# sovrasov/3d-object-detection.pytorch

Measured on AMD Instinct MI355X. Metric: regression train crops/sec @224^2 bs256 MobileNetV2, higher is better.
Workload: dtype bf16; 1 GPU; mobilenetv2 9-class Objectron keypoint regression, train step (fwd + l1/add/CE losses + bwd + AdamW), 224x224 crops, per-GPU batch 256; global_batch=256, parallelism=dp1, roofline_sampled_steps=0, rccl_ranks=0

## Files before the change

3d-object-detection.pytorch_amd/csrc/elementwise.hip:

```cpp
#include "common.h"

namespace {

template <typename T, bool U8>
__global__ __launch_bounds__(256) void im2col_kernel(const void* __restrict__ xin, const float* __restrict__ mean,
                                                     const float* __restrict__ istd, T* __restrict__ col, int B,
                                                     int H, int W, int Ho, int Wo) {
  extern __shared__ float tile[];
  const int WP = W + 2;
  const int hp = (Ho + 1) / 2;
  const int b = blockIdx.x / hp, oy0 = (blockIdx.x % hp) * 2;
  const int iy0 = oy0 * 2 - 1;
  const int tid = threadIdx.x;
  for (int i = tid; i < 15 * 2; i += 256) {
    const int rr = i >> 1;
    tile[rr * WP + ((i & 1) ? W + 1 : 0)] = 0.f;
  }
  if constexpr (U8) {
    const unsigned char* xu = reinterpret_cast<const unsigned char*>(xin);
    const float mu[3] = {mean[0], mean[1], mean[2]}, is[3] = {istd[0], istd[1], istd[2]};
    const int RB = W * 3;
    if ((RB & 3) == 0) {
      const int R4 = RB >> 2;
      for (int i = tid; i < 5 * R4; i += 256) {
// ... 245 lines not shown
template <typename T>
__global__ __launch_bounds__(256) void gap_fwd_kernel(const EwArgs a) {
  __shared__ float red[8 * 32 * 8];
  __shared__ float redm[8 * 32 * 8];
  __shared__ int redi[8 * 32 * 8];
  const int CG = a.C / 8, b = blockIdx.x;
  const int cgs = pool_cgs(CG), nslots = 256 / cgs, rowl = cgs * 8;
  const int cgl = threadIdx.x & (cgs - 1), slot = threadIdx.x / cgs;
  const int cg = blockIdx.y * cgs + cgl;
  const bool on = cg < CG;
  const int c0 = on ? cg * 8 : 0;
  const bool want_max = a.mode != T3D_POOL_AVG;
  const T* __restrict__ y = reinterpret_cast<const T*>(a.a);
  float sc[8], sh[8], acc[8], mx[8];
  int mi[8];
  load_affine(a, c0, sc, sh);
#pragma unroll
  for (int j = 0; j < 8; ++j) { acc[j] = 0.f; mx[j] = -INFINITY; mi[j] = 0; }
  if (on) {
    for (int hw = slot; hw < a.HW; hw += nslots) {
      float v[8];
      Vec8<T>::load(y + ((size_t)b * a.HW + hw) * a.C + c0, v);
      act_affine_vec<8>(v, sc, sh, a.act);
#pragma unroll
      for (int j = 0; j < 8; ++j) {
        acc[j] += v[j];
        if (v[j] > mx[j]) { mx[j] = v[j]; mi[j] = hw; }
      }
    }
  }
#pragma unroll
// ... 203 lines not shown
  else return T3D_ERR_ARG;
  T3D_CHECK_LAUNCH();
  return T3D_OK;
}

extern "C" int t3d_pool_fwd(int dtype, const void* y, const t3d_prologue* pro, int mode, float* pooled, int* argmax,
                            int B, int HW, int C, void* stream) {
  if (!y || !pooled || B <= 0 || HW <= 0 || C <= 0 || (C % 8)) return T3D_ERR_ARG;
  if (mode != T3D_POOL_AVG && mode != T3D_POOL_MAX && mode != T3D_POOL_AVGMAX) return T3D_ERR_ARG;
  if (pro && pro->se) return T3D_ERR_UNSUPPORTED;
  EwArgs a{};
  a.a = y; a.pooled = pooled; a.C = C; a.HW = HW; a.inv_hw = 1.f / (float)HW; a.mode = mode; a.argmax = argmax;
  fill_pro(a, pro);
  dim3 grid(B, cdiv(C / 8, 32));
  hipStream_t st = reinterpret_cast<hipStream_t>(stream);
  if (const int rc = t3d_fold_fallback(a.scale, st)) return rc;
  if (dtype == T3D_F32) T3D_LAUNCH(gap_fwd_kernel<float>, grid, dim3(256), 0, st, a);
  else if (dtype == T3D_BF16) T3D_LAUNCH(gap_fwd_kernel<bf16_t>, grid, dim3(256), 0, st, a);
  else if (dtype == T3D_F16) T3D_LAUNCH(gap_fwd_kernel<f16_t>, grid, dim3(256), 0, st, a);
  else return T3D_ERR_ARG;
  T3D_CHECK_LAUNCH();
  return T3D_OK;
}

extern "C" int t3d_gap_fwd(int dtype, const void* y, const t3d_prologue* pro, float* pooled, int B, int HW, int C,
                           void* stream) {
  return t3d_pool_fwd(dtype, y, pro, T3D_POOL_AVG, pooled, nullptr, B, HW, C, stream);
}

extern "C" int t3d_pool_bwd(int dtype, const float* dpooled, const void* y, const t3d_prologue* pro, int mode,
                            const int* argmax, void* dz, double* stats, int B, int HW, int C, void* stream) {
// ... 22 lines not shown
```

3d-object-detection.pytorch_amd/csrc/plan.hip:

```cpp
#include <chrono>
#include <cstdio>
#include <cstdlib>
#include <cstring>
#include <string>
#include <utility>
#include <vector>

#include "common.h"

namespace {

template <class T>
inline T word_to(uint64_t v) {
  if constexpr (std::is_pointer<T>::value) {
    return reinterpret_cast<T>(static_cast<uintptr_t>(v));
  } else if constexpr (std::is_same<T, float>::value) {
    const uint32_t b = static_cast<uint32_t>(v);
    float f;
    std::memcpy(&f, &b, 4);
    return f;
  } else if constexpr (std::is_same<T, double>::value) {
    double d;
    std::memcpy(&d, &v, 8);
    return d;
// ... 12 lines not shown

template <auto Fn>
struct Thunk;
template <class... A, int (*Fn)(A...)>
struct Thunk<Fn> {
  static int run(const uint64_t* w) { return call_words(Fn, w, std::index_sequence_for<A...>{}); }
};

struct Entry { const char* name; int (*run)(const uint64_t*); int nargs; };
#define T3D_E(fn) {#fn, &Thunk<&fn>::run, arity(&fn)}
const Entry kEntries[] = {
    T3D_E(t3d_dwconv_fwd), T3D_E(t3d_bn_finalize), T3D_E(t3d_bn_eval_affine), T3D_E(t3d_bn_eval_affine_batched),
    T3D_E(t3d_pwconv_fwd), T3D_E(t3d_pwconv_dgrad), T3D_E(t3d_pack_weight), T3D_E(t3d_sum_replicas_batched),
    T3D_E(t3d_set_dw_slots), T3D_E(t3d_set_exact_pool), T3D_E(t3d_sum_slots_batched), T3D_E(t3d_dwconv_bwd),
    T3D_E(t3d_pwconv_wgrad), T3D_E(t3d_pwconv_yfree_prep), T3D_E(t3d_pwconv_dgrad_yfree), T3D_E(t3d_pwconv_wgrad_yfree),
    T3D_E(t3d_pwconv_yfree_prep2), T3D_E(t3d_pwconv_bwd_yfree), T3D_E(t3d_pwconv_bwd_yfree_w), T3D_E(t3d_pwconv_wgrad_yfree_finish),
    T3D_E(t3d_bn_bwd_finalize), T3D_E(t3d_stem_im2col), T3D_E(t3d_stem_im2col_u8), T3D_E(t3d_crop_resize_u8),
    T3D_E(t3d_pwconv_fwd_mat), T3D_E(t3d_im2col), T3D_E(t3d_im2col_nchw), T3D_E(t3d_col2im_bwd), T3D_E(t3d_pack_conv_weight),
    T3D_E(t3d_unpack_conv_grad), T3D_E(t3d_maxpool_fwd), T3D_E(t3d_maxpool_bwd), T3D_E(t3d_res_relu_fwd),
    T3D_E(t3d_res_relu_bwd), T3D_E(t3d_subsample), T3D_E(t3d_ir_block_eval), T3D_E(t3d_bn_apply), T3D_E(t3d_bn_act_bwd),
    T3D_E(t3d_gap_fwd), T3D_E(t3d_gap_bwd), T3D_E(t3d_pool_fwd), T3D_E(t3d_pool_bwd), T3D_E(t3d_head_fwd),
    T3D_E(t3d_linear_fwd), T3D_E(t3d_head_fwd_all), T3D_E(t3d_head_bwd), T3D_E(t3d_head_bwd_weights), T3D_E(t3d_se_fwd),
    T3D_E(t3d_se_bwd), T3D_E(t3d_se_fwd_fused), T3D_E(t3d_se_bwd_data), T3D_E(t3d_se_bwd_weights), T3D_E(t3d_se_after_sums),
    T3D_E(t3d_se_after_apply), T3D_E(t3d_se_after_bwd), T3D_E(t3d_set_reduction_replicas), T3D_E(t3d_set_workspace), T3D_E(t3d_set_main_workspace),
    T3D_E(t3d_fold_request), T3D_E(t3d_pack_weights_batched), T3D_E(t3d_pwconv_pack_frag), T3D_E(t3d_adamw_step), T3D_E(t3d_set_grad_watch),
    T3D_E(t3d_sgd_step), T3D_E(t3d_rmsprop_step), T3D_E(t3d_adadelta_step),
    T3D_E(t3d_zero_batched), T3D_E(t3d_copy_cols), T3D_E(t3d_bn_bias_grad), T3D_E(t3d_se_bwd_affine), T3D_E(t3d_dropout_mask),
    T3D_E(t3d_loss_fwd_bwd), T3D_E(t3d_metrics_per_sample), T3D_E(t3d_iou3d), T3D_E(t3d_box_iou3d), T3D_E(t3d_ssd_decode_nms),
    T3D_E(t3d_expdw_fwd), T3D_E(t3d_track_step), T3D_E(t3d_ssd_select_rects), T3D_E(t3d_head_select), T3D_E(t3d_track_kp_to_frame),
};
// ... 247 lines not shown
```

3d-object-detection.pytorch_amd/csrc/pwconv_common.h:

```cpp
#pragma once
#include "common.h"

namespace t3d_pw {

struct GemmArgs {
  const void* a0;
  const void* a1;
  const float *p0, *p1, *p2;
  int act, se_after, per_sample, dgrad;
  const void* w;
  const float* bias;
  const void* e_y;
  const float *e_scale, *e_shift, *e_se;
  int e_act, e_se_after;
  const void* e_res;
  void* out;
  double* stats;
  float* ps_stats;
  int ps_wave;
  int M, HW, Kin, Nout, mtiles;
  int kz;
  float* part;
  const void* a2;
  int Kin2, ks1;
  int row0;
  const T3dFold* fold;
  const void* z_res;
  void* z_out;
  int unused_[8];
  int wfrag;
  T3dQuant quant;
};

template <typename T> __device__ __forceinline__ void ldvec(const T* p, float* v);
template <> __device__ __forceinline__ void ldvec<float>(const float* p, float* v) {
  const float4 a = *reinterpret_cast<const float4*>(p);
  v[0] = a.x; v[1] = a.y; v[2] = a.z; v[3] = a.w;
}
template <> __device__ __forceinline__ void ldvec<bf16_t>(const bf16_t* p, float* v) { Vec8<bf16_t>::load(p, v); }
template <typename T> __device__ __forceinline__ void stvec(T* p, const float* v);
template <> __device__ __forceinline__ void stvec<float>(float* p, const float* v) {
  *reinterpret_cast<float4*>(p) = make_float4(v[0], v[1], v[2], v[3]);
}
template <> __device__ __forceinline__ void stvec<bf16_t>(bf16_t* p, const float* v) { Vec8<bf16_t>::store(p, v); }
// ... 10 lines not shown
```

3d-object-detection.pytorch_amd/csrc/pwconv_stream.hip:

```cpp
#include <cstdlib>
#include <type_traits>
#include "pwconv_common.h"

#ifndef T3D_PW_F16
typedef bf16_t ST;
typedef bf16x8 ST8;
#define T3D_PW_MFMA __builtin_amdgcn_mfma_f32_16x16x32_bf16
#define T3D_PW_LAUNCH stream_launch
#else
typedef f16_t ST;
typedef f16x8 ST8;
#define T3D_PW_MFMA __builtin_amdgcn_mfma_f32_16x16x32_f16
#define T3D_PW_LAUNCH stream_launch_f16
#endif

namespace t3d_pw {
__device__ __forceinline__ f32x2 pk_fma_clamp01(f32x2 a, f32x2 b, f32x2 c) {
  f32x2 d;
  asm("v_pk_fma_f32 %0, %1, %2, %3 clamp" : "=v"(d) : "v"(a), "v"(b), "v"(c));
  return d;
}

namespace {


#ifdef T3D_PW_TRACE
__device__ unsigned long long g_pw_trace[16];
#define PW_STAMP(i)                                                                                       \
  do {                                                                                                    \
    if (threadIdx.x == 0 && (blockIdx.x == 0 || blockIdx.x == gridDim.x - 1))                            \
      g_pw_trace[(blockIdx.x == 0 ? 0 : 8) + (i)] = wall_clock64();                                       \
  } while (0)
#else
#define PW_STAMP(i)
#endif

template <int NT, int R, bool DG, bool GEN, bool YF = false, int KU = 2, bool ZM = false>
__global__ __launch_bounds__(512, KU > 2 ? 1 : 2) void pw_stream_kernel(const GemmArgs a, const int nchunks, const int KS, const int nrep, const long long rstride) {
  constexpr int BN = NT * 16;
  extern __shared__ __attribute__((aligned(16))) unsigned char smem[];
  ST8* Wf = reinterpret_cast<ST8*>(smem);
  const int kpad = KS * 32;
  float* coef = reinterpret_cast<float*>(smem + (size_t)NT * KS * 1024);
  float* lstat = coef + 3 * kpad;
  float* ecoef = lstat + BN * 2;
  double* dstat = reinterpret_cast<double*>(ecoef + 2 * BN);

  const int tid = threadIdx.x, lane = tid & 63, wave = tid >> 6;
  const int lg = lane >> 4, lc = lane & 15;
  const int nxb = gridDim.x / nchunks;
  int chunk, xb;
  if (nchunks > 1 && (nxb & 7) == 0) {
    const int xcd = blockIdx.x & 7, j = blockIdx.x >> 3;
    chunk = j % nchunks;
    xb = (j / nchunks) * 8 + xcd;
  } else {
    chunk = blockIdx.x % nchunks;
    xb = blockIdx.x / nchunks;
  }
  const int n0 = chunk * BN;
  const ST* __restrict__ A0 = reinterpret_cast<const ST*>(a.a0);
  const ST* __restrict__ A1 = reinterpret_cast<const ST*>(a.a1);
  const ST* __restrict__ A2 = reinterpret_cast<const ST*>(a.a2);
  const int ks1 = A2 ? a.ks1 : (1 << 30);
  const ST* __restrict__ Wg = reinterpret_cast<const ST*>(a.w);
  ST* __restrict__ out = reinterpret_cast<ST*>(a.out);
  PW_STAMP(0);

  const int nthr = blockDim.x, WAVES = nthr >> 6;
  auto stage_weights = [&]() {
  if (a.wfrag) {
    constexpr int SU = 8;
    const int total = NT * KS * 64, tiles = (a.Nout + 31) / 32 * 2, t0 = n0 / 16;
    const ST8* __restrict__ P = reinterpret_cast<const ST8*>(a.w) + (size_t)t0 * KS * 64;
    const int valid = max(0, min(NT, tiles - t0)) * KS * 64;
    for (int i0 = tid; i0 < total; i0 += nthr * SU) {
      ST8 v[SU];
#pragma unroll
      for (int u = 0; u < SU; ++u) v[u] = P[min(i0 + u * nthr, valid - 1)];
#pragma unroll
      for (int u = 0; u < SU; ++u) {
        const int i = i0 + u * nthr;
        if (i >= valid) {
#pragma unroll
// ... 14 lines not shown
        const int l = i & 63, ks = (i >> 6) % KS, t = (i >> 6) / KS;
        const int n = n0 + (t >> 1) * 32 + ((l & 15) >> 2) * 8 + (t & 1) * 4 + (l & 3), k = ks * 32 + (l >> 4) * 8;
        ok[u] = n < a.Nout && k < a.Kin;
        v[u] = *reinterpret_cast<const ST8*>(Wg + (size_t)min(n, a.Nout - 1) * a.Kin + min(k, a.Kin - 8));
      }
#pragma unroll
      for (int u = 0; u < SU; ++u) {
        if (!ok[u]) {
#pragma unroll
          for (int j = 0; j < 8; ++j) v[u][j] = (ST)0.f;
        }
        if (i0 + u * nthr < total) Wf[i0 + u * nthr] = v[u];
      }
    }
  }
  for (int i = tid; i < BN * 2; i += nthr) { lstat[i] = 0.f; dstat[i] = 0.0; }
  for (int i = tid; i < BN; i += nthr) {
    const int n = n0 + i;
    const bool v = DG && a.e_scale && n < a.Nout;
    ecoef[i] = v ? a.e_scale[n] : 1.f;
    ecoef[BN + i] = v ? a.e_shift[n] : 0.f;
  }
  };
  constexpr bool DGL = DG && !YF;
  if (!YF && a.fold) {
    for (int i = a.Kin + tid; i < kpad; i += nthr) {
      coef[i] = DG ? 0.f : 1.f; coef[kpad + i] = 0.f; coef[2 * kpad + i] = 0.f;
    }
    t3d_fold_block(a.fold, 0, a.Kin, coef, kpad, blockIdx.x == 0, stage_weights);
  } else {
  stage_weights();
  for (int i = tid; i < kpad; i += nthr) {
    const bool v = i < a.Kin;
    if (YF) {
      coef[i] = 1.f; coef[kpad + i] = 0.f; coef[2 * kpad + i] = 0.f;
    } else if (!DG) {
      coef[i] = (v && a.p0) ? a.p0[i] : 1.f;
      coef[kpad + i] = (v && a.p0) ? a.p1[i] : 0.f;
    } else {
      coef[i] = (v && !a.per_sample) ? a.p0[i] : 0.f;
// ... 220 lines not shown
            err[q] = *reinterpret_cast<const ST8*>(reinterpret_cast<const ST*>(a.e_res) + (size_t)mld[r] * a.Nout +
                                                      min(nb + 32 * q, a.Nout - 8));
        }
      }
#pragma unroll
      for (int q = 0; q < NT / 2; ++q) {
        const int n = nb + 32 * q;
        if (n >= a.Nout) continue;
        float v[8], yv[8];
#pragma unroll
        for (int j = 0; j < 8; ++j) v[j] = acc[r][2 * q + (j >> 2)][j & 3];
        if (c6f) {
#pragma unroll
          for (int j = 0; j < 8; ++j) v[j] *= 6.f;
        }
        if ((!DG || YF) && a.bias) {
#pragma unroll
          for (int j = 0; j < 8; ++j) v[j] += a.bias[n + j];
        }
        if (DG && a.e_y) {
#pragma unroll
          for (int j = 0; j < 8; ++j) yv[j] = (float)eyr[q][j];
          if (GEN && a.e_se) {
            const float4 s0 = *reinterpret_cast<const float4*>(ecoef + (n - n0)), s1 = *reinterpret_cast<const float4*>(ecoef + (n - n0) + 4);
            const float4 h0 = *reinterpret_cast<const float4*>(ecoef + BN + (n - n0)),
                         h1 = *reinterpret_cast<const float4*>(ecoef + BN + (n - n0) + 4);
            float es[8] = {s0.x, s0.y, s0.z, s0.w, s1.x, s1.y, s1.z, s1.w};
            float eh[8] = {h0.x, h0.y, h0.z, h0.w, h1.x, h1.y, h1.z, h1.w};
            const float4 g0 = esg[GEN ? q : 0][0], g1 = esg[GEN ? q : 0][1];
            const float sv[8] = {g0.x, g0.y, g0.z, g0.w, g1.x, g1.y, g1.z, g1.w};
            if (!a.e_se_after) {
// ... 93 lines not shown
        if (lc == 0 && n < a.Nout) {
          atomicAdd(dstat + (n - n0 + j) * 2, t3d_snap(s1, a.quant, false));
          atomicAdd(dstat + (n - n0 + j) * 2 + 1, t3d_snap(s2, a.quant, !DG));
        }
      }
    }
    __syncthreads();
    for (int i = tid; i < BN * 2; i += nthr) {
      const int n = n0 + (i >> 1);
      if (n < a.Nout) atomicAdd(a.stats + (size_t)(xb % nrep) * rstride + (size_t)(i & 1) * a.Nout + n, dstat[i]);
    }
  }
  PW_STAMP(4);
}

template <int NT, int R, bool DG, bool GEN, bool YF = false, int KU = 2, bool ZM = false>
int launch_v(GemmArgs& a, int KS, hipStream_t st) {
  constexpr int BN = NT * 16;
  const int kpad = KS * 32;
  const size_t lds = (size_t)NT * KS * 1024 + (size_t)3 * kpad * 4 + BN * 4 * 4 + BN * 2 * 8;
  if (lds > 150 * 1024) return T3D_ERR_UNSUPPORTED;
  const int nchunks = cdiv(a.Nout, BN);
  const int ngroups = cdiv(a.M, 16 * R);
  const bool ps = GEN && a.ps_stats != nullptr;
  const int gps = cdiv(a.HW, 16 * R);
  const int threads = (lds <= 48 * 1024 || (ps && gps <= 4)) ? 256 : 512;
  const void* fn = (const void*)pw_stream_kernel<NT, R, DG, GEN, YF, KU, ZM>;
  if (lds > 64 * 1024) (void)t3d_max_lds(fn, (int)lds);
  static int occ_cache[2] = {0, 0};
  int& occ = occ_cache[threads == 512];
  if (occ == 0) {
    int n = 0;
    if (hipOccupancyMaxActiveBlocksPerMultiprocessor(&n, fn, threads, 0) != hipSuccess || n < 1) n = 1;
    occ = n;
  }
  int per_cu = occ;
  const int by_lds = (int)(160 * 1024 / (lds + 512));
  if (per_cu > by_lds) per_cu = by_lds;
  if (per_cu < 1) per_cu = 1;
  int nxb = (256 * per_cu) / nchunks;
  a.ps_wave = (ps && gps <= 16) ? 1 : 0;
  const int need = ps ? (a.ps_wave ? cdiv(a.M / a.HW, threads / 64) : a.M / a.HW) : cdiv(ngroups, threads / 64);
  if (nxb > need) nxb = need;
  if (nxb < 1) nxb = 1;
  if (nchunks > 1 && nxb >= 8) {
    const int up = (nxb + 7) & ~7;
    nxb = (up * nchunks <= 256 * per_cu) ? up : (nxb & ~7);
  }
  a.quant = (!DG && a.stats && !T3D_ENV_SET("T3D_NO_SNAP")) ? t3d_quant_for(a.M) : T3dQuant{0.0, 0.0};
  if (YF || a.per_sample) {
    if (const int rc = t3d_fold_fallback(a.p0, st)) return rc;
    a.fold = nullptr;
  } else {
    a.fold = t3d_take_fold(a.p0);
  }
  T3D_LAUNCH_TIMED((pw_stream_kernel<NT, R, DG, GEN, YF, KU, ZM>), dim3(nxb * nchunks), dim3(threads), lds, st, a, nchunks, KS,
                     g_t3d_reduce.nrep, g_t3d_reduce.stats_stride);
  T3D_CHECK_LAUNCH();
  return T3D_OK;
}

template <int NT, int R>
int launch_nt(GemmArgs& a, int KS, hipStream_t st, int deep_ku = 0) {
#ifdef T3D_PW_F16
  if (a.a2 || a.dgrad || a.z_out || a.per_sample || a.ps_stats || a.e_se || a.stats) return T3D_ERR_UNSUPPORTED;
  if (a.p2) return launch_v<NT, R, false, true>(a, KS, st);
  return launch_v<NT, R, false, false>(a, KS, st);
#else
  if (a.a2) return launch_v<NT, R, true, false, true>(a, KS, st);
  const bool gen = a.per_sample || a.ps_stats || a.e_se || (!a.dgrad && a.p2);
  if (a.dgrad && !gen && deep_ku == 3) return launch_v<NT, R, true, false, false, 3>(a, KS, st);
  if (a.dgrad && !gen && deep_ku == 5) return launch_v<NT, R, true, false, false, 5>(a, KS, st);
  if (a.dgrad) return gen ? launch_v<NT, R, true, true>(a, KS, st) : launch_v<NT, R, true, false>(a, KS, st);
  if (a.z_out) return gen ? T3D_ERR_UNSUPPORTED : launch_v<NT, R, false, false, false, 2, true>(a, KS, st);
  return gen ? launch_v<NT, R, false, true>(a, KS, st) : launch_v<NT, R, false, false>(a, KS, st);
#endif
}

}

#if defined(T3D_PW_TRACE) && !defined(T3D_PW_F16)
extern "C" int t3d_debug_pw_trace(unsigned long long* out) {
  return hipMemcpyFromSymbol(out, HIP_SYMBOL(g_pw_trace), sizeof(unsigned long long) * 16) == hipSuccess ? 0 : -1;
// ... 47 lines not shown
```

3d-object-detection.pytorch_amd/csrc/pwconv_yfree.hip:

```cpp
#include "pwconv_common.h"

int t3d_pw_wgrad_tr_yfree(const void* dz, const void* x, float* tmp, int M, int HW, int K, int N, hipStream_t st);
size_t t3d_pw_bwd_yfree_scratch(int M, int K, int N);
int t3d_pw_bwd_yfree_launch(const void* dz, const void* x, const void* wd, const void* wt, const t3d_bnbwd* bb, const void* x_raw,
                            const void* residual, void* dx, double* stats, void* scratch, int M, int HW, int K, int N, hipStream_t st);
int t3d_pw_bwd_yfree_reduce(void* scratch, float** tmp_out, int M, int K, int N, hipStream_t st);

namespace {

__global__ __launch_bounds__(256) void yfree_prep_kernel(const bf16_t* __restrict__ wt, const float* __restrict__ alpha_g,
                                                         const float* __restrict__ beta_g, const float* __restrict__ gamma_g,
                                                         bf16_t* __restrict__ wcat, float* __restrict__ cvec, int K, int N,
                                                         int NP, int KP, const T3dFold* __restrict__ fold,
                                                         bf16_t* __restrict__ wd, int PBw) {
  extern __shared__ float fco[];
  __shared__ f32x4 red[3][64];
  const int t = threadIdx.x, lane = t & 63, wave = t >> 6, lg = lane >> 4, lc = lane & 15;
  if (fold) {
    t3d_fold_block(fold, 0, N, fco, N, blockIdx.x == 0 && blockIdx.y == 0);
  } else {
    for (int i = t; i < N; i += 256) { fco[i] = alpha_g[i]; fco[N + i] = beta_g[i]; fco[2 * N + i] = gamma_g[i]; }
    __syncthreads();
  }
  const float *alpha = fco, *beta = fco + N, *gamma = fco + 2 * N;
// ... 159 lines not shown
                     reinterpret_cast<bf16_t*>(wcat), cvec, K, N, rup32(N), rup32(K), fold, reinterpret_cast<bf16_t*>(wd), PBw);
  T3D_CHECK_LAUNCH();
  return T3D_OK;
}

extern "C" int t3d_pwconv_dgrad_yfree(const void* dz, const void* x, const void* wcat, const float* cvec,
                                      const void* x_raw, const t3d_prologue* pro_in, const void* residual, void* dx,
                                      double* stats, int M, int HW, int K, int N, void* stream) {
  if (!dz || !x || !wcat || !cvec || !dx || M <= 0 || HW <= 0 || K <= 0 || N <= 0 || (K % 8) || (N % 8)) return T3D_ERR_ARG;
  if (pro_in && pro_in->se) return T3D_ERR_UNSUPPORTED;
  t3d_pw::GemmArgs a{};
  a.dgrad = 1;
  a.a0 = dz; a.row0 = N;
  a.a2 = x; a.Kin2 = K; a.ks1 = rup32(N) / 32;
  a.w = wcat; a.bias = cvec; a.e_res = residual; a.out = dx; a.stats = stats;
  if (x_raw) {
    a.e_y = x_raw;
    if (pro_in) { a.e_scale = pro_in->scale; a.e_shift = pro_in->shift; a.e_act = pro_in->act; }
  }
  a.M = M; a.HW = HW; a.Kin = rup32(N) + rup32(K); a.Nout = K;
  return t3d_pw::stream_launch(a, reinterpret_cast<hipStream_t>(stream));
}

extern "C" int t3d_pwconv_wgrad_yfree(const void* dz, const void* x, const t3d_bnbwd* bb, const void* w, float* dw,
                                      int M, int HW, int K, int N, void* stream) {
  if (!dz || !x || !bb || !bb->alpha || !bb->beta || !bb->gamma || !w || !dw || M <= 0 || HW <= 0 || K <= 0 || N <= 0 ||
      (K % 8) || (N % 8))
    return T3D_ERR_ARG;
  if (bb->per_sample) return T3D_ERR_UNSUPPORTED;
  const size_t tmp_bytes = (size_t)(N + K + 8) * K * sizeof(float);
// ... 14 lines not shown
```

3d-object-detection.pytorch_amd/torchdet3d/_native.py:

```python
import ctypes
import os

import torch

_HERE = os.path.dirname(os.path.abspath(__file__))
LIB_PATH = os.environ.get('T3D_LIB') or os.path.join(os.path.dirname(_HERE), 'libt3d_hip.so')

W_FRAG = 0x100
F32, BF16, F16 = 0, 1, 2
ACT = {'none': 0, 'relu': 1, 'relu6': 2, 'hswish': 3}
POOL = {'avg': 0, 'max': 1, 'avg+max': 2}
_P, _I, _F, _D, _L = ctypes.c_void_p, ctypes.c_int, ctypes.c_float, ctypes.c_double, ctypes.c_longlong


class BnBwd(ctypes.Structure):
    _fields_ = [('alpha', _P), ('beta', _P), ('gamma', _P), ('per_sample', _I)]


class Prologue(ctypes.Structure):
    _fields_ = [('scale', _P), ('shift', _P), ('se', _P), ('act', _I), ('se_after_act', _I)]


class LossCfg(ctypes.Structure):
    _fields_ = [(n, _F) for n in ('c_l1', 'c_mse', 'c_smoothl1', 'smoothl1_beta', 'c_add', 'c_diag', 'c_wing',
# ... 17 lines not shown
    't3d_bn_eval_affine': [_I, _P, _P, _P, _P, _F, _P, _P, _P],
    't3d_bn_eval_affine_batched': [_P, _I, _F, _P],
    't3d_pwconv_fwd': [_I, _P, _PP, _P, _P, _P, _P, _I, _I, _I, _I, _P],
    't3d_pwconv_dgrad': [_I, _P, _P, _BP, _P, _P, _PP, _P, _P, _P, _P, _I, _I, _I, _I, _P],
    't3d_pack_weight': [_I, _P, _P, _I, _I, _I, _P],
    't3d_sum_replicas_batched': [_P, _I, _I, _P],
    't3d_set_dw_slots': [_I, _P],
    't3d_set_exact_pool': [_I],
    't3d_set_launch_events': [_P, _P],
    't3d_sum_slots_batched': [_P, _I, _P],
    't3d_dwconv_bwd': [_I, _P, _P, _BP, _P, _P, _PP, _P, _P, _P, _P, _I, _I, _I, _I, _I, _I, _P],
    't3d_pwconv_wgrad': [_I, _P, _P, _BP, _P, _PP, _P, _I, _I, _I, _I, _P],
    't3d_pwconv_yfree_prep': [_P, _BP, _P, _P, _I, _I, _P],
    't3d_pwconv_dgrad_yfree': [_P, _P, _P, _P, _P, _PP, _P, _P, _P, _I, _I, _I, _I, _P],
    't3d_pwconv_wgrad_yfree': [_P, _P, _BP, _P, _P, _I, _I, _I, _I, _P],
    't3d_pwconv_yfree_prep2': [_P, _BP, _P, _P, _P, _I, _I, _P],
    't3d_pwconv_bwd_yfree_scratch': [_I, _I, _I],
    't3d_pwconv_bwd_yfree': [_P, _P, _P, _P, _PP, _P, _P, _P, _P, _L, _I, _I, _I, _I, _P],
    't3d_pwconv_bwd_yfree_w': [_P, _P, _P, _BP, _P, _PP, _P, _P, _P, _P, _L, _I, _I, _I, _I, _P],
    't3d_pwconv_wgrad_yfree_finish': [_P, _BP, _P, _P, _I, _I, _I, _P],
    't3d_bn_bwd_finalize': [_P, _I, _D, _P, _P, _P, _P, _P, _P, _P, _P, _P],
    't3d_stem_im2col': [_I, _P, _P, _I, _I, _I, _P],
    't3d_stem_im2col_u8': [_I, _P, _P, _P, _P, _I, _I, _I, _P],
    't3d_crop_resize_u8': [_P, _P, _P, _I, _I, _I, _I, _I, _P],
    't3d_augment_crops_u8': [_P, _L, _P, _P, _I, _I, _I, _P],
    't3d_augment_resized_u8': [_P, _L, _P, _P, _I, _I, _I, _P],
    't3d_pwconv_fwd_mat': [_I, _P, _PP, _P, _P, _P, _P, _P, _I, _I, _I, _I, _P],
    't3d_ssd_decode_nms': [_I, _I, _P, _P, _P, _P, _P, _P, _P, _I, _I, _F, _F, _I, _F, _F, _P, _P, _P, _P],
    't3d_track_state_bytes': [_I],
    't3d_track_lds_bytes': [_I, _I],
# ... 131 lines not shown

    def summary(self):
        torch.cuda.synchronize()
        out = {}
        for name, nbytes, e0, e1 in self.rec:
            d = out.setdefault(name, dict(launches=0, ms=0.0, bytes=0))
            d['launches'] += 1
            d['ms'] += e0.elapsed_time(e1)
            d['bytes'] += nbytes or 0
        return out


timer = None
_KERNEL_TIMED = frozenset(('t3d_dwconv_fwd', 't3d_dwconv_bwd', 't3d_expdw_fwd', 't3d_pwconv_fwd', 't3d_pwconv_fwd_mat', 't3d_pwconv_dgrad',
                           't3d_pwconv_wgrad', 't3d_pwconv_dgrad_yfree', 't3d_pwconv_wgrad_yfree', 't3d_pwconv_bwd_yfree',
                           't3d_pwconv_bwd_yfree_w'))
_ABLATE = frozenset(x for x in os.environ.get('T3D_ABLATE', '').split(',') if x)


SLOT_IMGS, SLOT_GT, SLOT_CATS, SLOT_DROPOUT, SLOT_STEP, SLOT_LR, SLOT_RB_DST, SLOT_RB_EVENT, NSLOTS = range(9)
recorder = None


def call(name, *args, nbytes=None, slots=None):
    if _ABLATE and name in _ABLATE:
        return
    fn = getattr(lib(), name)
    if recorder is not None:
        recorder.add_call(name, args, nbytes, slots)
        rc = fn(*args)
        recorder.after_call()
# ... 144 lines not shown
```

3d-object-detection.pytorch_amd/torchdet3d/models/engine.py:

```python
import math
import os

import torch

from .. import _native as N
from .arch import Arch

BN_EPS, BN_MOM = 1e-5, 0.1
NREP = 16
FUSED_EVAL_MIN_B = int(os.environ.get('T3D_FUSED_EVAL_MIN_B', '96'))
DW_SLOTS = int(os.environ.get('T3D_DW_SLOTS', '512'))
WORKSPACE_BYTES = 64 << 20
MAIN_WORKSPACE_BYTES = 16 << 20
YFREE_MIN_ELEMS = int(os.environ.get('T3D_YFREE_MIN', 8 << 20))
YFREE_MAX_K = int(os.environ.get('T3D_YFREE_MAX_K', 112))
HOOK_MIN = 1 << 20
SE_AFTER_FUSED = None
HOOK_ON_SIDE = True


def _se_after_fused_by_shape(dt, B, HW, C, R):
    if B < 8:
        return False
    if C * R <= 4096:
# ... 340 lines not shown
            f.gamma = N.ptr(bn.gamma)
            if which == 0:
                f.stats, f.beta, f.rm, f.rv, f.nbt = N.ptr(bn.stats), N.ptr(bn.beta), N.ptr(bn.rm), N.ptr(bn.rv), N.ptr(bn.nbt)
                f.momentum, f.eps = BN_MOM, BN_EPS
                f.o0, f.o1, f.o2, f.o3 = N.ptr(bn.scale), N.ptr(bn.shift), N.ptr(bn.mean), N.ptr(bn.invstd)
            else:
                f.stats, f.mean, f.invstd = N.ptr(bn.bstats), N.ptr(bn.mean), N.ptr(bn.invstd)
                f.o0, f.o1, f.o2 = N.ptr(bn.alpha), N.ptr(bn.bbeta), N.ptr(bn.gammac)
                f.o3, f.o4 = N.ptr(bn.dgamma), N.ptr(bn.dbeta)
            host = torch.frombuffer(bytearray(bytes(f)), dtype=torch.uint8)
            d = bn.desc[key] = host.to(self.device)
        return d

    _LAZY_DW = '1'
    DERIVING = frozenset(('t3d_pwconv_fwd', 't3d_pwconv_fwd_mat', 't3d_bn_apply', 't3d_pool_fwd', 't3d_pwconv_dgrad', 't3d_pwconv_yfree_prep',
                          't3d_pwconv_bwd_yfree_w', 't3d_se_bwd_affine')
                         + (('t3d_dwconv_fwd',) if _LAZY_DW in ('1', 'fwd') else ())
                         + (('t3d_dwconv_bwd',) if _LAZY_DW in ('1', 'bwd') else ()))

    def _c(self, entry, *args, fwd=None, bwd=None, **kw):
        req = False
        if fwd is not None and fwd.pend[0]:
            if self._lazy and entry in self.DERIVING:
                N.call('t3d_fold_request', N.ptr(self._fold_desc(fwd, 0, fwd.count)), N.ptr(fwd.scale))
                fwd.pend[0], req = False, True
            else:
                self._settle_f(fwd)
        if bwd is not None and bwd.pend[1]:
            if self._lazy and entry in self.DERIVING and not req:
                N.call('t3d_fold_request', N.ptr(self._fold_desc(bwd, 1, bwd.count)), N.ptr(bwd.alpha))
                bwd.pend[1], req = False, True
# ... 625 lines not shown
            self.grad_hook(lo)

    def _se_after_fused(self, B, HW, C, R):
        if self.arch.keys.scheme != 'timm' or C > 1024 or R > 1024:
            return False
        if SE_AFTER_FUSED is not None:
            return bool(SE_AFTER_FUSED)
        return _se_after_fused_by_shape(self.dt, B, HW, C, R)

    def _yfree_ok(self, x, M, K, Nn):
        return (self.dt == N.BF16 and YFREE_MIN_ELEMS > 0 and x.pro is None and K <= YFREE_MAX_K
                and M * Nn >= YFREE_MIN_ELEMS)

    def _expand_bwd_yfree(self, d1, bb1, bn1, wname, x, res, M, K, Nn, i):
        st = N.stream()
        tot = (Nn + 31) // 32 * 32 + (K + 31) // 32 * 32
        wcat = self._buf(f'wcat:{i}', (K, tot))
        cvec = self._buf(f'cvec:{i}', (K,), torch.float32)
        HW = x.H * x.W
        with_stats = x.bn is not None and not x.finished_act
        need = N.lib().t3d_pwconv_bwd_yfree_scratch(M, K, Nn) if not (with_stats and x.gpro is not None) else 0
        if need > 0:
            scratch = self._buf(f'yfscr:{i}', (need,), torch.uint8)
            dx = self._buf(f'dzin:{i}', (M, K))
            self._c('t3d_pwconv_bwd_yfree_w', N.ptr(d1), N.ptr(x.t), N.ptr(self.wt[wname]), bb1, N.ptr(x.raw) if with_stats else None,
                    None, N.ptr(res) if res is not None else None, N.ptr(dx), self._bst(x.bn) if with_stats else None,
                    N.ptr(scratch), need, M, HW, K, Nn, st, nbytes=M * (K + Nn) * self.esz, bwd=bn1)
            self._wgrad(N.ptr(scratch), bb1, N.ptr(self.w[wname]), N.ptr(self.g[wname]), M, K, Nn, entry='t3d_pwconv_wgrad_yfree_finish')
            if x.finished_act:
                dx = self._act_bwd(dx, x, f'dzin:{i}:a')
            return dx
        self._c('t3d_pwconv_yfree_prep', N.ptr(self.wt[wname]), bb1, N.ptr(wcat), N.ptr(cvec), K, Nn, st, bwd=bn1)
        self._wgrad(N.ptr(d1), N.ptr(x.t), bb1, N.ptr(self.w[wname]), N.ptr(self.g[wname]), M, HW, K, Nn,
                    entry='t3d_pwconv_wgrad_yfree', nbytes=M * (K + Nn) * self.esz)
        dx = self._buf(f'dzin:{i}', (M, K))
        N.call('t3d_pwconv_dgrad_yfree', N.ptr(d1), N.ptr(x.t), N.ptr(wcat), N.ptr(cvec),
               N.ptr(x.raw) if with_stats else None, x.gpro if with_stats else None,
               N.ptr(res) if res is not None else None, N.ptr(dx),
               self._bst(x.bn) if with_stats else None, M, HW, K, Nn, st, nbytes=M * (K + Nn) * self.esz)
        if x.finished_act:
            dx = self._act_bwd(dx, x, f'dzin:{i}:a')
        return dx

    def _act_bwd(self, dz, x, tag):
        M = x.B * x.H * x.W
        out = self._buf(tag, (M, x.C))
        N.call('t3d_bn_act_bwd', self.dt, N.ptr(dz), N.ptr(x.raw), x.gpro, N.ptr(out), self._bst(x.bn), M, x.C,
               N.stream())
        return out

    def _block_bwd(self, rec, dz):
        st, dt = N.stream(), self.dt
        blk, i, x, src, s2 = rec['blk'], rec['idx'], rec['x'], rec['src'], rec['s2']
        dwn, pwn = rec['names']
# ... 108 lines not shown
```

include/t3d.h:

```cpp
#ifndef T3D_H_
#define T3D_H_
#include <stdint.h>
#ifdef __cplusplus
extern "C" {
#endif

enum { T3D_F32 = 0, T3D_BF16 = 1, T3D_F16 = 2 };
enum { T3D_W_FRAG = 0x100 };
enum { T3D_ACT_NONE = 0, T3D_ACT_RELU = 1, T3D_ACT_RELU6 = 2, T3D_ACT_HSWISH = 3 };
enum { T3D_OK = 0, T3D_ERR_ARG = -1, T3D_ERR_LAUNCH = -2, T3D_ERR_UNSUPPORTED = -3 };

typedef struct {
  const float* scale;
  const float* shift;
  const float* se;
  int act;
  int se_after_act;
} t3d_prologue;

int t3d_version(void);

int t3d_dwconv_fwd(int dtype, const void* x, const t3d_prologue* pro, const float* w, void* y,
                   double* stats, float* gap_sum, int B, int H, int W, int C, int k, int stride,
                   void* stream);
// ... 27 lines not shown
                     double* stats, float* ps_stats, int M, int HW, int K, int N, void* stream);

int t3d_sum_replicas_batched(const long long* desc, int n, int nrep, void* stream);

int t3d_pack_weight(int dtype, const float* w, void* out, int rows, int cols, int transpose, void* stream);

int t3d_pwconv_wgrad(int dtype, const void* dz, const void* y, const t3d_bnbwd* bb, const void* x,
                     const t3d_prologue* pro, float* dw, int M, int HW, int K, int N, void* stream);

int t3d_pwconv_yfree_prep(const void* wt, const t3d_bnbwd* bb, void* wcat, float* cvec, int K, int N, void* stream);
int t3d_pwconv_dgrad_yfree(const void* dz, const void* x, const void* wcat, const float* cvec, const void* x_raw,
                           const t3d_prologue* pro_in, const void* residual, void* dx, double* stats, int M, int HW,
                           int K, int N, void* stream);
int t3d_pwconv_wgrad_yfree(const void* dz, const void* x, const t3d_bnbwd* bb, const void* w, float* dw, int M, int HW,
                           int K, int N, void* stream);

int t3d_pwconv_yfree_prep2(const void* wt, const t3d_bnbwd* bb, void* wcat, float* cvec, void* wd, int K, int N, void* stream);
int t3d_pwconv_bwd_yfree_w(const void* dz, const void* x, const void* wt, const t3d_bnbwd* bb, const void* x_raw,
                           const t3d_prologue* pro_in, const void* residual, void* dx, double* stats, void* scratch,
                           long long scratch_bytes, int M, int HW, int K, int N, void* stream);
int t3d_pwconv_bwd_yfree_scratch(int M, int K, int N);
int t3d_pwconv_bwd_yfree(const void* dz, const void* x, const void* wd, const void* x_raw, const t3d_prologue* pro_in,
                         const void* residual, void* dx, double* stats, void* scratch, long long scratch_bytes, int M, int HW,
                         int K, int N, void* stream);
int t3d_pwconv_wgrad_yfree_finish(void* scratch, const t3d_bnbwd* bb, const void* w, float* dw, int M, int K, int N, void* stream);

int t3d_dwconv_bwd(int dtype, const void* dz, const void* y, const t3d_bnbwd* bb, const float* w,
                   const void* x, const t3d_prologue* pro, const void* residual, void* dx, double* stats,
                   float* dw, int B, int H, int W, int C, int k, int stride, void* stream);

// ... 229 lines not shown
```

Measured before the change: 38520 crops/s.

## Fuse y-free dgrad weight prep into the streaming kernel and fold BN in pool

Adds a YB variant of the pointwise streaming kernel. Each block builds its own concatenated weight fragment (alpha-scaled W, the W·diag(beta)·Wᵀ product via MFMA) and the gamma bias in LDS, so the separate t3d_pwconv_yfree_prep launch and its wcat/cvec global buffers are no longer needed. The engine now calls the new dgrad_yfree_w entry before wgrad. The global-average-pool forward also consumes pending BN folds inside the kernel instead of forcing a fallback launch. In exchange, every block redundantly recomputes the weight product, which adds per-block prologue work and LDS use.

```diff
diff --git a/3d-object-detection.pytorch_amd/csrc/elementwise.hip b/3d-object-detection.pytorch_amd/csrc/elementwise.hip
--- a/3d-object-detection.pytorch_amd/csrc/elementwise.hip
+++ b/3d-object-detection.pytorch_amd/csrc/elementwise.hip
@@ -283,7 +283,15 @@
   const T* __restrict__ y = reinterpret_cast<const T*>(a.a);
   float sc[8], sh[8], acc[8], mx[8];
   int mi[8];
-  load_affine(a, c0, sc, sh);
+  if (a.fold) {
+    __shared__ float fco[2 * 32 * 8];
+    const int cb0 = blockIdx.y * rowl, c0l = on ? cgl * 8 : 0;
+    t3d_fold_block(a.fold, cb0, min(rowl, a.C - cb0), fco, rowl, blockIdx.x == 0);
+#pragma unroll
+    for (int i = 0; i < 8; ++i) { sc[i] = fco[c0l + i]; sh[i] = fco[rowl + c0l + i]; }
+  } else {
+    load_affine(a, c0, sc, sh);
+  }
 #pragma unroll
   for (int j = 0; j < 8; ++j) { acc[j] = 0.f; mx[j] = -INFINITY; mi[j] = 0; }
   if (on) {
@@ -517,7 +525,7 @@
   fill_pro(a, pro);
   dim3 grid(B, cdiv(C / 8, 32));
   hipStream_t st = reinterpret_cast<hipStream_t>(stream);
-  if (const int rc = t3d_fold_fallback(a.scale, st)) return rc;
+  a.fold = t3d_take_fold(a.scale);
   if (dtype == T3D_F32) T3D_LAUNCH(gap_fwd_kernel<float>, grid, dim3(256), 0, st, a);
   else if (dtype == T3D_BF16) T3D_LAUNCH(gap_fwd_kernel<bf16_t>, grid, dim3(256), 0, st, a);
   else if (dtype == T3D_F16) T3D_LAUNCH(gap_fwd_kernel<f16_t>, grid, dim3(256), 0, st, a);
diff --git a/3d-object-detection.pytorch_amd/csrc/plan.hip b/3d-object-detection.pytorch_amd/csrc/plan.hip
--- a/3d-object-detection.pytorch_amd/csrc/plan.hip
+++ b/3d-object-detection.pytorch_amd/csrc/plan.hip
@@ -50,6 +50,7 @@
     T3D_E(t3d_pwconv_fwd), T3D_E(t3d_pwconv_dgrad), T3D_E(t3d_pack_weight), T3D_E(t3d_sum_replicas_batched),
     T3D_E(t3d_set_dw_slots), T3D_E(t3d_set_exact_pool), T3D_E(t3d_sum_slots_batched), T3D_E(t3d_dwconv_bwd),
     T3D_E(t3d_pwconv_wgrad), T3D_E(t3d_pwconv_yfree_prep), T3D_E(t3d_pwconv_dgrad_yfree), T3D_E(t3d_pwconv_wgrad_yfree),
+    T3D_E(t3d_pwconv_dgrad_yfree_w),
     T3D_E(t3d_pwconv_yfree_prep2), T3D_E(t3d_pwconv_bwd_yfree), T3D_E(t3d_pwconv_bwd_yfree_w), T3D_E(t3d_pwconv_wgrad_yfree_finish),
     T3D_E(t3d_bn_bwd_finalize), T3D_E(t3d_stem_im2col), T3D_E(t3d_stem_im2col_u8), T3D_E(t3d_crop_resize_u8),
     T3D_E(t3d_pwconv_fwd_mat), T3D_E(t3d_im2col), T3D_E(t3d_im2col_nchw), T3D_E(t3d_col2im_bwd), T3D_E(t3d_pack_conv_weight),
diff --git a/3d-object-detection.pytorch_amd/csrc/pwconv_common.h b/3d-object-detection.pytorch_amd/csrc/pwconv_common.h
--- a/3d-object-detection.pytorch_amd/csrc/pwconv_common.h
+++ b/3d-object-detection.pytorch_amd/csrc/pwconv_common.h
@@ -27,7 +27,8 @@
   const T3dFold* fold;
   const void* z_res;
   void* z_out;
-  int unused_[8];
+  int yf_build;
+  int unused_[7];
   int wfrag;
   T3dQuant quant;
 };
diff --git a/3d-object-detection.pytorch_amd/csrc/pwconv_stream.hip b/3d-object-detection.pytorch_amd/csrc/pwconv_stream.hip
--- a/3d-object-detection.pytorch_amd/csrc/pwconv_stream.hip
+++ b/3d-object-detection.pytorch_amd/csrc/pwconv_stream.hip
@@ -35,7 +35,7 @@
 #define PW_STAMP(i)
 #endif
 
-template <int NT, int R, bool DG, bool GEN, bool YF = false, int KU = 2, bool ZM = false>
+template <int NT, int R, bool DG, bool GEN, bool YF = false, int KU = 2, bool ZM = false, bool YB = false>
 __global__ __launch_bounds__(512, KU > 2 ? 1 : 2) void pw_stream_kernel(const GemmArgs a, const int nchunks, const int KS, const int nrep, const long long rstride) {
   constexpr int BN = NT * 16;
   extern __shared__ __attribute__((aligned(16))) unsigned char smem[];
@@ -45,6 +45,7 @@
   float* lstat = coef + 3 * kpad;
   float* ecoef = lstat + BN * 2;
   double* dstat = reinterpret_cast<double*>(ecoef + 2 * BN);
+  float* cbias = reinterpret_cast<float*>(dstat + 2 * BN);
 
   const int tid = threadIdx.x, lane = tid & 63, wave = tid >> 6;
   const int lg = lane >> 4, lc = lane & 15;
@@ -68,6 +69,15 @@
   PW_STAMP(0);
 
   const int nthr = blockDim.x, WAVES = nthr >> 6;
+  auto stage_consts = [&]() {
+  for (int i = tid; i < BN * 2; i += nthr) { lstat[i] = 0.f; dstat[i] = 0.0; }
+  for (int i = tid; i < BN; i += nthr) {
+    const int n = n0 + i;
+    const bool v = DG && a.e_scale && n < a.Nout;
+    ecoef[i] = v ? a.e_scale[n] : 1.f;
+    ecoef[BN + i] = v ? a.e_shift[n] : 0.f;
+  }
+  };
   auto stage_weights = [&]() {
   if (a.wfrag) {
     constexpr int SU = 8;
@@ -112,16 +122,104 @@
       }
     }
   }
-  for (int i = tid; i < BN * 2; i += nthr) { lstat[i] = 0.f; dstat[i] = 0.0; }
-  for (int i = tid; i < BN; i += nthr) {
-    const int n = n0 + i;
-    const bool v = DG && a.e_scale && n < a.Nout;
-    ecoef[i] = v ? a.e_scale[n] : 1.f;
-    ecoef[BN + i] = v ? a.e_shift[n] : 0.f;
-  }
+  stage_consts();
   };
   constexpr bool DGL = DG && !YF;
-  if (!YF && a.fold) {
+  if constexpr (YB) {
+    const int Nz = a.row0, K = a.Nout, ks1b = a.ks1, KP = (KS - ks1b) * 32;
+    if (a.fold) {
+      t3d_fold_block(a.fold, 0, Nz, coef, kpad, blockIdx.x == 0);
+    } else {
+      for (int i = tid; i < Nz; i += nthr) { coef[i] = a.p0[i]; coef[kpad + i] = a.p1[i]; coef[2 * kpad + i] = a.p2[i]; }
+      __syncthreads();
+    }
+    const float *alpha = coef, *beta = coef + kpad, *gamma = coef + 2 * kpad;
+    {
+      constexpr int SU = 8;
+      const int total = NT * ks1b * 64;
+      for (int i0 = tid; i0 < total; i0 += nthr * SU) {
+        ST8 v[SU];
+#pragma unroll
+        for (int u = 0; u < SU; ++u) {
+          const int i = min(i0 + u * nthr, total - 1);
+          const int l = i & 63, ks = (i >> 6) % ks1b, t = (i >> 6) / ks1b;
+          const int k = n0 + (t >> 1) * 32 + ((l & 15) >> 2) * 8 + (t & 1) * 4 + (l & 3), n = ks * 32 + (l >> 4) * 8;
+          v[u] = *reinterpret_cast<const ST8*>(Wg + (size_t)min(k, K - 1) * Nz + min(n, Nz - 8));
+        }
+#pragma unroll
+        for (int u = 0; u < SU; ++u) {
+          const int i = i0 + u * nthr;
+          if (i < total) {
+            const int l = i & 63, ks = (i >> 6) % ks1b, t = (i >> 6) / ks1b;
+            const int k = n0 + (t >> 1) * 32 + ((l & 15) >> 2) * 8 + (t & 1) * 4 + (l & 3), n = ks * 32 + (l >> 4) * 8;
+            const bool ok = k < K && n < Nz;
+            const int nc = min(n, Nz - 8);
+            ST8 o;
+#pragma unroll
+            for (int j = 0; j < 8; ++j) o[j] = (ST)(ok ? alpha[nc + j] * (float)v[u][j] : 0.f);
+            Wf[(t * KS + ks) * 64 + l] = o;
+          }
+        }
+      }
+    }
+    {
+      ST* const Wfe = reinterpret_cast<ST*>(Wf);
+      const int nst = (Nz + 31) / 32, qtiles = KP / 16;
+      for (int un = wave; un < NT * qtiles; un += WAVES) {
+        const int kt = un / qtiles, qt = un % qtiles;
+        const int k0 = n0 + kt * 16, q0 = qt * 16;
+        f32x4 qa[4];
+#pragma unroll
+        for (int p = 0; p < 4; ++p) qa[p] = f32x4{0.f, 0.f, 0.f, 0.f};
+        if (k0 < KP) {
+          const ST* ra = Wg + (size_t)min(k0 + lc, K - 1) * Nz;
+          const ST* rb = Wg + (size_t)min(q0 + lc, K - 1) * Nz;
+          for (int s0 = 0; s0 < nst; s0 += 4) {
+            ST8 fa[4], fb[4];
+#pragma unroll
+            for (int p = 0; p < 4; ++p) {
+              const int nc = min((s0 + p) * 32 + 8 * lg, Nz - 8);
+              fa[p] = *reinterpret_cast<const ST8*>(ra + nc);
+              fb[p] = *reinterpret_cast<const ST8*>(rb + nc);
+            }
+#pragma unroll
+            for (int p = 0; p < 4; ++p) {
+              const int n = (s0 + p) * 32 + 8 * lg;
+              const bool live = n < Nz;
+              const int nc = min(n, Nz - 8);
+              ST8 b;
+#pragma unroll
+              for (int j = 0; j < 8; ++j) b[j] = (ST)(live ? beta[nc + j] * (float)fb[p][j] : 0.f);
+              qa[p] = T3D_PW_MFMA(fa[p], b, qa[p], 0, 0, 0);
+            }
+          }
+        }
+        f32x4 q = qa[0];
+        q += qa[1];
+        q += qa[2];
+        q += qa[3];
+#pragma unroll
+        for (int r = 0; r < 4; ++r) {
+          const int kl = kt * 16 + 4 * lg + r, k2 = q0 + lc;
+          const int t = (kl >> 5) * 2 + ((kl >> 2) & 1), l = ((k2 >> 3) & 3) * 16 + ((kl >> 3) & 3) * 4 + (kl & 3);
+          Wfe[(size_t)((t * KS + ks1b + (k2 >> 5)) * 64 + l) * 8 + (k2 & 7)] = (ST)((n0 + kl < K && k2 < K) ? q[r] : 0.f);
+        }
+      }
+    }
+    for (int kb = 0; kb < BN; kb += nthr / 16) {
+      const int row = tid >> 4, sub = tid & 15, k = n0 + kb + row;
+      float s2 = 0.f;
+      if (k < K)
+        for (int n = sub * 8; n < Nz; n += 128) {
+          const ST8 v = *reinterpret_cast<const ST8*>(Wg + (size_t)k * Nz + n);
+#pragma unroll
+          for (int j = 0; j < 8; ++j) s2 = fmaf(gamma[n + j], (float)v[j], s2);
+        }
+      s2 = row16_sum(s2);
+      if (sub == 0 && kb + row < BN) cbias[kb + row] = k < K ? s2 : 0.f;
+    }
+    stage_consts();
+  } else if (!YF && a.fold) {
     for (int i = a.Kin + tid; i < kpad; i += nthr) {
       coef[i] = DG ? 0.f : 1.f; coef[kpad + i] = 0.f; coef[2 * kpad + i] = 0.f;
     }
@@ -372,7 +470,10 @@
 #pragma unroll
           for (int j = 0; j < 8; ++j) v[j] *= 6.f;
         }
-        if ((!DG || YF) && a.bias) {
+        if constexpr (YB) {
+#pragma unroll
+          for (int j = 0; j < 8; ++j) v[j] += cbias[n - n0 + j];
+        } else if ((!DG || YF) && a.bias) {
 #pragma unroll
           for (int j = 0; j < 8; ++j) v[j] += a.bias[n + j];
         }
@@ -496,18 +597,18 @@
   PW_STAMP(4);
 }
 
-template <int NT, int R, bool DG, bool GEN, bool YF = false, int KU = 2, bool ZM = false>
+template <int NT, int R, bool DG, bool GEN, bool YF = false, int KU = 2, bool ZM = false, bool YB = false>
 int launch_v(GemmArgs& a, int KS, hipStream_t st) {
   constexpr int BN = NT * 16;
   const int kpad = KS * 32;
-  const size_t lds = (size_t)NT * KS * 1024 + (size_t)3 * kpad * 4 + BN * 4 * 4 + BN * 2 * 8;
+  const size_t lds = (size_t)NT * KS * 1024 + (size_t)3 * kpad * 4 + BN * 4 * 4 + BN * 2 * 8 + (YB ? BN * 4 : 0);
   if (lds > 150 * 1024) return T3D_ERR_UNSUPPORTED;
   const int nchunks = cdiv(a.Nout, BN);
   const int ngroups = cdiv(a.M, 16 * R);
   const bool ps = GEN && a.ps_stats != nullptr;
   const int gps = cdiv(a.HW, 16 * R);
   const int threads = (lds <= 48 * 1024 || (ps && gps <= 4)) ? 256 : 512;
-  const void* fn = (const void*)pw_stream_kernel<NT, R, DG, GEN, YF, KU, ZM>;
+  const void* fn = (const void*)pw_stream_kernel<NT, R, DG, GEN, YF, KU, ZM, YB>;
   if (lds > 64 * 1024) (void)t3d_max_lds(fn, (int)lds);
   static int occ_cache[2] = {0, 0};
   int& occ = occ_cache[threads == 512];
@@ -530,13 +631,13 @@
     nxb = (up * nchunks <= 256 * per_cu) ? up : (nxb & ~7);
   }
   a.quant = (!DG && a.stats && !T3D_ENV_SET("T3D_NO_SNAP")) ? t3d_quant_for(a.M) : T3dQuant{0.0, 0.0};
-  if (YF || a.per_sample) {
+  if ((YF && !YB) || a.per_sample) {
     if (const int rc = t3d_fold_fallback(a.p0, st)) return rc;
     a.fold = nullptr;
   } else {
     a.fold = t3d_take_fold(a.p0);
   }
-  T3D_LAUNCH_TIMED((pw_stream_kernel<NT, R, DG, GEN, YF, KU, ZM>), dim3(nxb * nchunks), dim3(threads), lds, st, a, nchunks, KS,
+  T3D_LAUNCH_TIMED((pw_stream_kernel<NT, R, DG, GEN, YF, KU, ZM, YB>), dim3(nxb * nchunks), dim3(threads), lds, st, a, nchunks, KS,
                      g_t3d_reduce.nrep, g_t3d_reduce.stats_stride);
   T3D_CHECK_LAUNCH();
   return T3D_OK;
@@ -549,6 +650,7 @@
   if (a.p2) return launch_v<NT, R, false, true>(a, KS, st);
   return launch_v<NT, R, false, false>(a, KS, st);
 #else
+  if (a.a2 && a.yf_build) return launch_v<NT, R, true, false, true, 2, false, true>(a, KS, st);
   if (a.a2) return launch_v<NT, R, true, false, true>(a, KS, st);
   const bool gen = a.per_sample || a.ps_stats || a.e_se || (!a.dgrad && a.p2);
   if (a.dgrad && !gen && deep_ku == 3) return launch_v<NT, R, true, false, false, 3>(a, KS, st);
diff --git a/3d-object-detection.pytorch_amd/csrc/pwconv_yfree.hip b/3d-object-detection.pytorch_amd/csrc/pwconv_yfree.hip
--- a/3d-object-detection.pytorch_amd/csrc/pwconv_yfree.hip
+++ b/3d-object-detection.pytorch_amd/csrc/pwconv_yfree.hip
@@ -197,6 +197,27 @@
   a.a0 = dz; a.row0 = N;
   a.a2 = x; a.Kin2 = K; a.ks1 = rup32(N) / 32;
   a.w = wcat; a.bias = cvec; a.e_res = residual; a.out = dx; a.stats = stats;
+  if (x_raw) {
+    a.e_y = x_raw;
+    if (pro_in) { a.e_scale = pro_in->scale; a.e_shift = pro_in->shift; a.e_act = pro_in->act; }
+  }
+  a.M = M; a.HW = HW; a.Kin = rup32(N) + rup32(K); a.Nout = K;
+  return t3d_pw::stream_launch(a, reinterpret_cast<hipStream_t>(stream));
+}
+
+extern "C" int t3d_pwconv_dgrad_yfree_w(const void* dz, const void* x, const void* wt, const t3d_bnbwd* bb, const void* x_raw,
+                                        const t3d_prologue* pro_in, const void* residual, void* dx, double* stats, int M,
+                                        int HW, int K, int N, void* stream) {
+  if (!dz || !x || !wt || !bb || !bb->alpha || !bb->beta || !bb->gamma || !dx || M <= 0 || HW <= 0 || K <= 0 || N <= 0 ||
+      (K % 8) || (N % 8))
+    return T3D_ERR_ARG;
+  if (bb->per_sample || (pro_in && pro_in->se)) return T3D_ERR_UNSUPPORTED;
+  t3d_pw::GemmArgs a{};
+  a.dgrad = 1;
+  a.a0 = dz; a.row0 = N;
+  a.a2 = x; a.Kin2 = K; a.ks1 = rup32(N) / 32;
+  a.w = wt; a.yf_build = 1; a.p0 = bb->alpha; a.p1 = bb->beta; a.p2 = bb->gamma;
+  a.e_res = residual; a.out = dx; a.stats = stats;
   if (x_raw) {
     a.e_y = x_raw;
     if (pro_in) { a.e_scale = pro_in->scale; a.e_shift = pro_in->shift; a.e_act = pro_in->act; }
diff --git a/3d-object-detection.pytorch_amd/torchdet3d/_native.py b/3d-object-detection.pytorch_amd/torchdet3d/_native.py
--- a/3d-object-detection.pytorch_amd/torchdet3d/_native.py
+++ b/3d-object-detection.pytorch_amd/torchdet3d/_native.py
@@ -55,6 +55,7 @@
     't3d_pwconv_yfree_prep': [_P, _BP, _P, _P, _I, _I, _P],
     't3d_pwconv_dgrad_yfree': [_P, _P, _P, _P, _P, _PP, _P, _P, _P, _I, _I, _I, _I, _P],
     't3d_pwconv_wgrad_yfree': [_P, _P, _BP, _P, _P, _I, _I, _I, _I, _P],
+    't3d_pwconv_dgrad_yfree_w': [_P, _P, _P, _BP, _P, _PP, _P, _P, _P, _I, _I, _I, _I, _P],
     't3d_pwconv_yfree_prep2': [_P, _BP, _P, _P, _P, _I, _I, _P],
     't3d_pwconv_bwd_yfree_scratch': [_I, _I, _I],
     't3d_pwconv_bwd_yfree': [_P, _P, _P, _P, _PP, _P, _P, _P, _P, _L, _I, _I, _I, _I, _P],
@@ -216,7 +217,7 @@
 timer = None
 _KERNEL_TIMED = frozenset(('t3d_dwconv_fwd', 't3d_dwconv_bwd', 't3d_expdw_fwd', 't3d_pwconv_fwd', 't3d_pwconv_fwd_mat', 't3d_pwconv_dgrad',
                            't3d_pwconv_wgrad', 't3d_pwconv_dgrad_yfree', 't3d_pwconv_wgrad_yfree', 't3d_pwconv_bwd_yfree',
-                           't3d_pwconv_bwd_yfree_w'))
+                           't3d_pwconv_bwd_yfree_w', 't3d_pwconv_dgrad_yfree_w'))
 _ABLATE = frozenset(x for x in os.environ.get('T3D_ABLATE', '').split(',') if x)
 
 
diff --git a/3d-object-detection.pytorch_amd/torchdet3d/models/engine.py b/3d-object-detection.pytorch_amd/torchdet3d/models/engine.py
--- a/3d-object-detection.pytorch_amd/torchdet3d/models/engine.py
+++ b/3d-object-detection.pytorch_amd/torchdet3d/models/engine.py
@@ -378,7 +378,7 @@
 
     _LAZY_DW = '1'
     DERIVING = frozenset(('t3d_pwconv_fwd', 't3d_pwconv_fwd_mat', 't3d_bn_apply', 't3d_pool_fwd', 't3d_pwconv_dgrad', 't3d_pwconv_yfree_prep',
-                          't3d_pwconv_bwd_yfree_w', 't3d_se_bwd_affine')
+                          't3d_pwconv_bwd_yfree_w', 't3d_pwconv_dgrad_yfree_w', 't3d_se_bwd_affine')
                          + (('t3d_dwconv_fwd',) if _LAZY_DW in ('1', 'fwd') else ())
                          + (('t3d_dwconv_bwd',) if _LAZY_DW in ('1', 'bwd') else ()))
 
@@ -1034,9 +1034,6 @@
 
     def _expand_bwd_yfree(self, d1, bb1, bn1, wname, x, res, M, K, Nn, i):
         st = N.stream()
-        tot = (Nn + 31) // 32 * 32 + (K + 31) // 32 * 32
-        wcat = self._buf(f'wcat:{i}', (K, tot))
-        cvec = self._buf(f'cvec:{i}', (K,), torch.float32)
         HW = x.H * x.W
         with_stats = x.bn is not None and not x.finished_act
         need = N.lib().t3d_pwconv_bwd_yfree_scratch(M, K, Nn) if not (with_stats and x.gpro is not None) else 0
@@ -1050,14 +1047,13 @@
             if x.finished_act:
                 dx = self._act_bwd(dx, x, f'dzin:{i}:a')
             return dx
-        self._c('t3d_pwconv_yfree_prep', N.ptr(self.wt[wname]), bb1, N.ptr(wcat), N.ptr(cvec), K, Nn, st, bwd=bn1)
+        dx = self._buf(f'dzin:{i}', (M, K))
+        self._c('t3d_pwconv_dgrad_yfree_w', N.ptr(d1), N.ptr(x.t), N.ptr(self.wt[wname]), bb1,
+                N.ptr(x.raw) if with_stats else None, x.gpro if with_stats else None,
+                N.ptr(res) if res is not None else None, N.ptr(dx),
+                self._bst(x.bn) if with_stats else None, M, HW, K, Nn, st, nbytes=M * (K + Nn) * self.esz, bwd=bn1)
         self._wgrad(N.ptr(d1), N.ptr(x.t), bb1, N.ptr(self.w[wname]), N.ptr(self.g[wname]), M, HW, K, Nn,
                     entry='t3d_pwconv_wgrad_yfree', nbytes=M * (K + Nn) * self.esz)
-        dx = self._buf(f'dzin:{i}', (M, K))
-        N.call('t3d_pwconv_dgrad_yfree', N.ptr(d1), N.ptr(x.t), N.ptr(wcat), N.ptr(cvec),
-               N.ptr(x.raw) if with_stats else None, x.gpro if with_stats else None,
-               N.ptr(res) if res is not None else None, N.ptr(dx),
-               self._bst(x.bn) if with_stats else None, M, HW, K, Nn, st, nbytes=M * (K + Nn) * self.esz)
         if x.finished_act:
             dx = self._act_bwd(dx, x, f'dzin:{i}:a')
         return dx
diff --git a/include/t3d.h b/include/t3d.h
--- a/include/t3d.h
+++ b/include/t3d.h
@@ -65,6 +65,9 @@
                            int K, int N, void* stream);
 int t3d_pwconv_wgrad_yfree(const void* dz, const void* x, const t3d_bnbwd* bb, const void* w, float* dw, int M, int HW,
                            int K, int N, void* stream);
+int t3d_pwconv_dgrad_yfree_w(const void* dz, const void* x, const void* wt, const t3d_bnbwd* bb, const void* x_raw,
+                             const t3d_prologue* pro_in, const void* residual, void* dx, double* stats, int M, int HW,
+                             int K, int N, void* stream);
 
 int t3d_pwconv_yfree_prep2(const void* wt, const t3d_bnbwd* bb, void* wcat, float* cvec, void* wd, int K, int N, void* stream);
 int t3d_pwconv_bwd_yfree_w(const void* dz, const void* x, const void* wt, const t3d_bnbwd* bb, const void* x_raw,
```

Result: slower. 37740 crops/s (-2.0%).
